# JuliaLinearAlgebra/IterativeSolvers.jl

Hardware: AMD Instinct MI355X
Metric: cg_iters_per_sec (higher is better)
Workload: dtype f64; 1 GPU; cg! on 256^3 3D 7-point Laplacian (test/laplace_matrix.jl), fp64, hashed rhs, x0 = 0 (BASELINE.json configs[1]); n=16777216, nnz=117047296

## Files before the change

iterativesolvers.jl_amd/csrc/mik_core.hip:

```cpp
#include <algorithm>
#include <cmath>
#include <cstdarg>
#include <limits>
#include <new>

#include "mik_kernels.h"
#include "mik_spmv.h"
#include <algorithm>
#include <mutex>

#include "mik_sell.h"
#include "mik_jds.h"
#include <map>
#include <string>
#include <unordered_map>

thread_local std::string g_mik_create_error;
int g_mik_tuning[MIK_KNOB_COUNT] = {0};
static std::vector<mik_ctx *> g_mik_contexts;
static std::mutex g_mik_contexts_mu;

int mik_fail(mik_ctx *ctx, int code, const char *fmt, ...)
{
    char buf[512];
// ... 877 lines not shown
    std::vector<int> rowptr, col;
    std::vector<unsigned char> v;
    if (ctx->tuning[MIK_KNOB_UPLOAD] != 1 && nnz > 0 && n_rows > 0 && n_cols > 0 && n_rows < 0x7f000000) {
        mik_csr *A = new (std::nothrow) mik_csr();
        if (!A) return mik_fail(ctx, MIK_ERR_NOMEM, "mik_csr_create: host allocation failed");
        A->ctx = ctx; A->dtype = dtype; A->n_rows = n_rows; A->n_cols = n_cols; A->nnz = nnz;
        (void)hipSetDevice(ctx->device);
        int rc = mik_upload_device(ctx, A, dtype, n_rows, n_cols, nnz, ptr, idx, val, index_base, is_csc);
        if (rc == MIK_OK && !A->sdia_val && !A->sdia_pats && (ctx->tuning[MIK_KNOB_LAYOUTS] & 1) == 0 && ctx->tuning[MIK_KNOB_UPLOAD] != 2) {
            rc = mik_build_sdiaw_device(ctx, A);
            if (rc == MIK_OK) rc = mik_build_jds_device(ctx, A);
            if (rc == MIK_OK) rc = mik_build_xwin_device(ctx, A);
        } else if (rc == MIK_OK && !A->sdia_val && !A->sdia_pats && (ctx->tuning[MIK_KNOB_LAYOUTS] & 1) == 0) {
            try {
                rowptr.resize((size_t)n_rows + 1);
                col.resize((size_t)nnz);
                v.resize((size_t)nnz * es);
            } catch (const std::bad_alloc &) {
                mik_csr_destroy(A);
                return mik_fail(ctx, MIK_ERR_NOMEM, "mik_csr_create: host staging allocation failed");
            }
            if (hipMemcpy(rowptr.data(), A->rowptr, sizeof(int) * ((size_t)n_rows + 1), hipMemcpyDeviceToHost) != hipSuccess ||
                hipMemcpy(col.data(), A->col, sizeof(int) * (size_t)nnz, hipMemcpyDeviceToHost) != hipSuccess ||
                hipMemcpy(v.data(), A->val, es * (size_t)nnz, hipMemcpyDeviceToHost) != hipSuccess) {
                mik_csr_destroy(A);
                return mik_fail(ctx, MIK_ERR_HIP, "mik_csr_create: reading the device CSR back failed");
            }
            rc = csr_build_sdiaw(ctx, A, rowptr, col, v, es, n_rows, n_cols, nnz);
            if (rc == MIK_OK) rc = csr_build_jds(ctx, A, rowptr, col, v, es, n_rows, nullptr);
            if (rc == MIK_OK) rc = csr_build_xwin(ctx, A, rowptr, col, es, n_rows, n_cols, A->max_row_nnz);
            if (rc == MIK_OK) rc = mik_build_rperm_host(ctx, A, rowptr.data());
        }
        if (rc == MIK_OK) rc = sdiaw_chunk_bits(ctx, A);
        if (rc == MIK_OK) { *out = A; return MIK_OK; }
        mik_csr_destroy(A);
        if (rc != MIK_ERR_NOTIMPL) return rc;
    }
    if (on_device) return MIK_ERR_NOTIMPL;
    try {
        rowptr.assign((size_t)n_rows + 1, 0);
        col.resize((size_t)nnz);
        v.resize((size_t)nnz * es);
    } catch (const std::bad_alloc &) {
        return mik_fail(ctx, MIK_ERR_NOMEM, "mik_csr_create: host staging allocation failed");
    }
    for (int64_t j = 0; j < n_major; ++j)
        if (ptr[j + 1] < ptr[j]) return mik_fail(ctx, MIK_ERR_INVALID, "mik_csr_create: ptr not monotone at %lld", (long long)j);
    for (int64_t k = 0; k < nnz; ++k) {
        const int64_t i = idx[k] - index_base;
        if (i < 0 || i >= n_minor) return mik_fail(ctx, MIK_ERR_INVALID, "mik_csr_create: index %lld out of range at %lld", (long long)idx[k], (long long)k);
    }
    int max_row = 0;
    if (is_csc) {
        for (int64_t k = 0; k < nnz; ++k) rowptr[(size_t)(idx[k] - index_base) + 1]++;
        for (int64_t r = 0; r < n_rows; ++r) {
            max_row = std::max(max_row, rowptr[r + 1]);
            rowptr[r + 1] += rowptr[r];
        }
        std::vector<int> cursor(rowptr.begin(), rowptr.end() - 1);
        for (int64_t j = 0; j < n_cols; ++j)
            for (int64_t k = ptr[j] - index_base; k < ptr[j + 1] - index_base; ++k) {
                const int64_t r = idx[k] - index_base;
                const int dst = cursor[r]++;
                col[dst] = (int)j;
                memcpy(&v[(size_t)dst * es], (const unsigned char *)val + (size_t)k * es, es);
            }
// ... 137 lines not shown
                for (size_t q = 4 * g2; q < std::min(4 * g2 + 4, long_rows.size()); ++q) {
                    lo = std::min<int64_t>(lo, col[(size_t)long_start[q]]);
                    hi = std::max<int64_t>(hi, col[(size_t)long_start[q] + (size_t)long_len[q] - 1]);
                }
                lo &= ~(int64_t)(W - 1);
                if (lo + LW > n_cols) lo = (n_cols - LW) & ~(int64_t)(W - 1);
                if (hi - lo < 2 * LW) { lwin[g2] = (int)lo; ++with_window; }
            }
            A->long_spread = 2 * with_window >= nwg;
            if (!A->long_spread) {
                std::fill(lwin.begin(), lwin.end(), -1);
                std::vector<int> ord(long_rows.size());
                for (size_t q = 0; q < ord.size(); ++q) ord[q] = (int)q;
                std::stable_sort(ord.begin(), ord.end(), [&](int a, int b) { return long_len[(size_t)a] > long_len[(size_t)b]; });
                std::vector<int> tab3;
                for (int q : ord) tab3.push_back(long_rows[(size_t)q]);
                for (int q : ord) tab3.push_back(long_start[(size_t)q]);
                for (int q : ord) tab3.push_back(long_len[(size_t)q]);
                if (hipMemcpy(A->long_rows, tab3.data(), sizeof(int) * tab3.size(), hipMemcpyHostToDevice) != hipSuccess) {
                    cleanup();
                    return mik_fail(ctx, MIK_ERR_HIP, "mik_csr_create: long-row table");
                }
            }
            hipError_t e2;
            if ((e2 = hipMalloc((void **)&A->long_win, sizeof(int) * nwg)) != hipSuccess ||
                (e2 = hipMemcpy(A->long_win, lwin.data(), sizeof(int) * nwg, hipMemcpyHostToDevice)) != hipSuccess) {
                cleanup();
                return mik_fail(ctx, MIK_ERR_HIP, "mik_csr_create: long-row windows: %s", hipGetErrorString(e2));
            }
            A->long_lw = (int)LW;
        }
    }
    if (rc_layout == MIK_OK) rc_layout = sdiaw_chunk_bits(ctx, A);
    if (rc_layout != MIK_OK) { cleanup(); return rc_layout; }
    *out = A;
    return MIK_OK;
}

extern "C" int mik_csr_destroy(mik_csr *A)
{
    if (!A) return MIK_OK;
    if (A->ctx) (void)hipStreamSynchronize(A->ctx->stream);
    if (A->rowptr) (void)hipFree(A->rowptr);
    if (A->col) (void)hipFree(A->col);
    if (A->val) (void)hipFree(A->val);
    if (A->long_rows) (void)hipFree(A->long_rows);
    if (A->is_long) (void)hipFree(A->is_long);
    if (A->seg_sum) (void)hipFree(A->seg_sum);
    if (A->sdia_ptr) (void)hipFree(A->sdia_ptr);
    if (A->sdia_off) (void)hipFree(A->sdia_off);
    if (A->sdia_tri) (void)hipFree(A->sdia_tri);
    if (A->sdia_mask) (void)hipFree(A->sdia_mask);
    if (A->sdia_val) (void)hipFree(A->sdia_val);
    if (A->sdia_pats) (void)hipFree(A->sdia_pats);
    if (A->sdia_pat_id) (void)hipFree(A->sdia_pat_id);
    if (A->sdia_recs) (void)hipFree(A->sdia_recs);
    if (A->sdiaw_pats) (void)hipFree(A->sdiaw_pats);
    if (A->sdiaw_pat_id) (void)hipFree(A->sdiaw_pat_id);
    if (A->sdiaw_mask) (void)hipFree(A->sdiaw_mask);
    if (A->sdiaw_uz) (void)hipFree(A->sdiaw_uz);
    if (A->xwin_lo) (void)hipFree(A->xwin_lo);
    if (A->rperm) (void)hipFree(A->rperm);
    if (A->long_win) (void)hipFree(A->long_win);
    if (A->jds_ptr) (void)hipFree(A->jds_ptr);
    if (A->jds_len) (void)hipFree(A->jds_len);
    if (A->jds_col) (void)hipFree(A->jds_col);
    if (A->jds_val) (void)hipFree(A->jds_val);
    delete A;
    return MIK_OK;
}

static int spmv_kernel_choice(const mik_csr *A);
extern "C" int mik_csr_layout(const mik_csr *A, int *layout)
{
    if (!A || !layout) return MIK_ERR_INVALID;
    *layout = spmv_kernel_choice(A);
// ... 33 lines not shown
    if (!A) return MIK_ERR_INVALID;
    if (n_rows) *n_rows = A->n_rows;
    if (n_cols) *n_cols = A->n_cols;
    if (nnz) *nnz = A->nnz;
    if (dtype) *dtype = A->dtype;
    return MIK_OK;
}

template <typename T>
int mik_spmv_launch_range(mik_ctx *ctx, const mik_csr *A, const T *x, T *y, bool fuse_dot, T *seg_out, const int *done, int rb_begin,
                          int rb_count);

static int spmv_kernel_choice(const mik_csr *A)
{
    const bool csr = A->col != nullptr;
    if (A->force_layout == 0 && csr) return 0;
    if ((A->ctx->tuning[MIK_KNOB_LAYOUTS] & 1) == 0 || !csr) {
        if (A->sdia_pats && ((A->ctx->tuning[MIK_KNOB_LAYOUTS] & 4) == 0 || !csr)) return 5;
        if (A->sdia_val && ((A->ctx->tuning[MIK_KNOB_LAYOUTS] & 4) == 0 || !csr)) return 4;
        if (A->sdiaw_pats && ((A->ctx->tuning[MIK_KNOB_LAYOUTS] & 4) == 0 || !csr)) return 6;
        if (A->jds_val && (A->ctx->tuning[MIK_KNOB_LAYOUTS] & 8) == 0) return 1;
    }
    return 0;
}

extern "C" int mik_csr_compact(mik_csr *A)
{
    if (!A) return MIK_ERR_INVALID;
    if (!A->col) return MIK_OK;
    if (!(A->sdia_pats || A->sdia_val || A->sdiaw_pats || A->jds_val) || A->n_long)
        return mik_fail(A->ctx, MIK_ERR_NOTIMPL, "mik_csr_compact: this operator runs on its CSR arrays");
    if (A->ctx) { (void)hipSetDevice(A->ctx->device); (void)hipStreamSynchronize(A->ctx->stream); }
    (void)hipFree(A->rowptr); (void)hipFree(A->col); (void)hipFree(A->val);
    A->rowptr = nullptr; A->col = nullptr; A->val = nullptr;
    return MIK_OK;
}

static inline bool spmv_csr_rowgather(const mik_csr *A)
{
    return A->ctx->tuning[MIK_KNOB_CSR_KERNEL] == 2 || (A->ctx->tuning[MIK_KNOB_CSR_KERNEL] == 0 && A->n_long == 0 && !A->xwin_lo && !A->rperm);
}

static bool sdiab2_applies(const mik_csr *A)
{
    return A->sdia_buf_ok && A->sdia_cls >= 1 && (A->n_rows & 1) == 0 && A->ctx->tuning[MIK_KNOB_SDIA_KERNEL] == 0;
}

bool mik_spmv_has_epilogue(const mik_csr *A)
{
    if (!A || A->ctx->tuning[MIK_KNOB_SOLVER_FORM] == 2) return false;
    const int kc = spmv_kernel_choice(A);
    if (kc == 5) return A->sdia_buf_ok && A->ctx->tuning[MIK_KNOB_SDIA_KERNEL] != 1 && sdiab2_applies(A);
    return (kc == 0 || kc == 1) && A->n_long == 0;
}

bool mik_spmv_is_light(const mik_csr *A) { return A && (spmv_kernel_choice(A) == 5 || spmv_kernel_choice(A) == 6); }

extern "C" int mik_spmv_kernel(const mik_csr *A, char *name, int len)
{
    if (!A || !name || len <= 0) return MIK_ERR_INVALID;
    const char *k = "k_spmv_rowblock";
    switch (spmv_kernel_choice(A)) {
    case 5: k = A->sdia_buf_ok && A->ctx->tuning[MIK_KNOB_SDIA_KERNEL] != 1 ? (sdiab2_applies(A) ? "k_spmv_sdiab2" : "k_spmv_sdiab") : "k_spmv_sdiac"; break;
    case 6: k = ((A->n_rows & 1) == 0 && A->ctx->tuning[MIK_KNOB_SDIA_KERNEL] != 3) ? "k_spmv_sdiaw2" : "k_spmv_sdiaw"; break;
    case 4: k = "k_spmv_sdia"; break;
    case 1: k = "k_spmv_jds"; break;
    default: k = spmv_csr_rowgather(A) ? "k_spmv_rowgather" : ((A->xwin_lo && (A->ctx->tuning[MIK_KNOB_LAYOUTS] & 96) == 0) ? "k_spmv_rowblock+xwin" : "k_spmv_rowblock"); break;
// ... 157 lines not shown
        lt.seg_sum = A->seg_sum; lt.nlong = nlong;
    }
    const int nlb = (nlong + 3) / 4;
    const int *lwin = (A->long_win && (ctx->tuning[MIK_KNOB_LAYOUTS] & 96) == 0 && mik_aligned16(x)) ? A->long_win : nullptr;
    if (choice == 1) {
        using IV = typename WideVec<T>::idx;
        using VV = typename WideVec<T>::val;
        const bool inside = fuse_dot && nlong == 0;
#define MIK_JDS_GO(FD, NTV, MG)                                                                                                        \
    hipLaunchKernelGGL((k_spmv_jds<T, FD, NTV, MG>), dim3(nb + (MG ? nlb : 0)), dim3(MIK_BLOCK), 0, ctx->stream, n, rb0, A->jds_ptr, A->jds_len, \
                       (const IV *)A->jds_col, (const VV *)A->jds_val, x, y, seg_out, done, nlb, lt, A->col, (const T *)A->val, (const T *)ctx->spmv_ep_w, (const T *)ctx->spmv_ep_c, (const T *)ctx->spmv_ep_z)
#define MIK_JDS_GO2(NTV)                                                                      \
    do {                                                                                      \
        if (inside) MIK_JDS_GO(true, NTV, false);                                             \
        else if (nlong) MIK_JDS_GO(false, NTV, true);                                         \
        else MIK_JDS_GO(false, NTV, false);                                                   \
    } while (0)
        MIK_JDS_GO2(true);
#undef MIK_JDS_GO2
#undef MIK_JDS_GO
        MIK_LAUNCH_CHECK(ctx);
        if (fuse_dot && !inside) {
            hipLaunchKernelGGL((k_rowdot<T>), dim3(nb_all), dim3(MIK_BLOCK), 0, ctx->stream, n, x, (const T *)y, seg_out, done);
            MIK_LAUNCH_CHECK(ctx);
        }
        return MIK_OK;
    }
    if (spmv_csr_rowgather(A)) {
        if (nlong) {
            hipLaunchKernelGGL((k_spmv_longrows<T>), dim3(nlb), dim3(MIK_BLOCK), lwin ? sizeof(T) * (size_t)A->long_lw : 0, ctx->stream, lt, A->col, (const T *)A->val, x, y, done,
                               lwin, A->long_lw);
            MIK_LAUNCH_CHECK(ctx);
        }
#define MIK_RG_GO(FD, NTV)                                                                                                      \
    hipLaunchKernelGGL((k_spmv_rowgather<T, FD, NTV>), dim3(nb), dim3(MIK_BLOCK), 0, ctx->stream, n, rb0, nb, map_mode, A->rowptr, \
                       A->col, (const T *)A->val, x, y, seg_out, done, A->is_long, (const T *)ctx->spmv_ep_w, (const T *)ctx->spmv_ep_c, (const T *)ctx->spmv_ep_z)
        if (fuse_dot) { MIK_RG_GO(true, true); }
        else          { MIK_RG_GO(false, true); }
#undef MIK_RG_GO
        MIK_LAUNCH_CHECK(ctx);
        return MIK_OK;
    }
    const bool merge = nlong > 0 && !fuse_dot;
    const bool nt_rb = !A->xwin_lo;
    if (nlong && !merge) {
        hipLaunchKernelGGL((k_spmv_longrows<T>), dim3(nlb), dim3(MIK_BLOCK), lwin ? sizeof(T) * (size_t)A->long_lw : 0, ctx->stream, lt, A->col, (const T *)A->val, x, y, done,
                           lwin, A->long_lw);
        MIK_LAUNCH_CHECK(ctx);
    }
    const dim3 grid(nb + (merge ? nlb : 0)), block(MIK_BLOCK);
    const bool xwin = A->xwin_lo && wide && (ctx->tuning[MIK_KNOB_LAYOUTS] & 96) == 0 && mik_aligned16(x);
    constexpr int RB_TILE = MIK_SPMV_TILE * (int)(8 / sizeof(T));
    const size_t dyn = sizeof(T) * ((size_t)RB_TILE + 12 + (xwin ? (size_t)A->xwin_span : 0));
    const int lw_launch = (int)std::min<size_t>((size_t)A->long_lw, dyn / 1024 * (1024 / sizeof(T)));
    const bool rp = A->rperm && wide && (ctx->tuning[MIK_KNOB_LAYOUTS] & 96) == 0;
#define MIK_SPMV_GO(FD, NT, WD, MG, XW, RP)                                                                      \
    hipLaunchKernelGGL((k_spmv_rowblock<T, FD, NT, WD, MG, XW, RP>), grid, block, dyn, ctx->stream, n, nb, map_mode, A->rowptr, \
                       A->col, (const T *)A->val, x, y, seg_out, done, A->is_long, nlb, lt, (const int *)A->xwin_lo, A->xwin_span, (const unsigned char *)A->rperm, \
                       MG ? lwin : (const int *)nullptr, (MG && lwin && A->long_spread) ? -lw_launch : lw_launch, (const T *)ctx->spmv_ep_w, (const T *)ctx->spmv_ep_c, (const T *)ctx->spmv_ep_z)
#define MIK_SPMV_GO3(FD, NT, MG)                                                          \
    do {                                                                                  \
        if (xwin) { if (rp) MIK_SPMV_GO(FD, NT, true, MG, true, true); else MIK_SPMV_GO(FD, NT, true, MG, true, false); }   \
        else if (rp) MIK_SPMV_GO(FD, NT, true, MG, false, true);                          \
        else if (wide) MIK_SPMV_GO(FD, NT, true, MG, false, false);                       \
        else MIK_SPMV_GO(FD, NT, false, MG, false, false);                                \
    } while (0)
#define MIK_SPMV_GO2(FD, MG) do { if (nt_rb) MIK_SPMV_GO3(FD, true, MG); else MIK_SPMV_GO3(FD, false, MG); } while (0)
    if (fuse_dot) MIK_SPMV_GO2(true, false);
// ... 357 lines not shown
```

iterativesolvers.jl_amd/csrc/mik_internal.h:

```cpp
#pragma once
#include <hip/hip_runtime.h>

#include <algorithm>
#include <cmath>
#include <cstdint>
#include <cstdio>
#include <cstring>
#include <limits>
#include <string>
#include <vector>

#include "../../include/mik.h"
#include "../../include/mik_dev.h"

constexpr int MIK_BLOCK = 256;
constexpr int MIK_RED_L = 2;
constexpr int MIK_FIN_THREADS = 1024;
constexpr int MIK_SPMV_TILE = 2048;
constexpr int MIK_SPMV_G = 1;
constexpr int MIK_LONG_ROW = 256;
constexpr int MIK_XCD_MAP = 8;

template <typename T> struct VT;
template <> struct VT<double> { static constexpr int W = 2; using vec = double2; };
// ... 18 lines not shown
    const void *spmv_ep_w = nullptr, *spmv_ep_c = nullptr;
    const void *spmv_ep_z = nullptr;
    int tuning[MIK_KNOB_COUNT] = {0};
    static constexpr size_t COEF_BYTES = 8192;
    static constexpr size_t COEF_SAFE_SLOT = 4096;
    std::vector<std::pair<void *, int (*)(void *)>> owned;
};

static inline int mik_cus(const mik_ctx *ctx) { const int v = ctx->tuning[MIK_KNOB_MACHINE] & 0xFFFF; return v > 0 ? v : std::max(1, ctx->cu_count); }
static inline int mik_xcds(const mik_ctx *ctx) { const int v = (ctx->tuning[MIK_KNOB_MACHINE] >> 16) & 0xFF; return v > 0 ? v : std::max(1, ctx->xcd_count); }
static inline bool mik_xcd_maps(const mik_ctx *ctx) { return mik_xcds(ctx) == MIK_XCD_MAP; }
static inline int mik_max_grid(const mik_ctx *ctx) { return mik_cus(ctx) * 32; }
static inline int mik_resident_cap(const mik_ctx *ctx) { return mik_cus(ctx); }
static inline int mik_strip_for(const mik_ctx *ctx, int64_t bw, int64_t nb)
{
    if (!mik_xcd_maps(ctx)) return 0;
    const int64_t P = ((bw + MIK_BLOCK - 1) / MIK_BLOCK + MIK_XCD_MAP - 1) / MIK_XCD_MAP * MIK_XCD_MAP;
    return (P >= MIK_XCD_MAP && P <= nb / 4) ? (int)P : 0;
}

int mik_mgs_resident_max_s();

struct mik_csr {
    mik_ctx *ctx = nullptr;
    int dtype = MIK_F64;
    int64_t n_rows = 0, n_cols = 0, nnz = 0;
    int *rowptr = nullptr;
    int *col = nullptr;
    void *val = nullptr;
    int max_row_nnz = 0;
    int strip = 0;
    int force_layout = -1;
    int max_rowblock_nnz = 0;
    int n_long = 0;
    int *xwin_lo = nullptr;
    int xwin_span = 0;
    int *long_win = nullptr;
    int long_lw = 0;
    bool long_spread = false;
    unsigned char *rperm = nullptr;
    int *long_rows = nullptr;
    int n_seg = 0, n_cut = 0;
    void *seg_sum = nullptr;
    unsigned char *is_long = nullptr;
    void *sdiaw_pats = nullptr;
    int *sdiaw_pat_id = nullptr;
    unsigned *sdiaw_mask = nullptr;
    void *sdiaw_uz = nullptr;
    int sdiaw_npat = 0, sdiaw_koff = 0, sdiaw_pat_bytes = 0;
    int *jds_ptr = nullptr;
    unsigned short *jds_len = nullptr;
    int *jds_col = nullptr;
    void *jds_val = nullptr;
    int64_t jds_groups = 0;
    int64_t jds_short_nnz = 0;
    int *sdia_ptr = nullptr;
    int *sdia_off = nullptr;
    int *sdia_tri = nullptr;
    unsigned char *sdia_mask = nullptr;
    void *sdia_val = nullptr;
    int64_t sdia_entries = 0;
    void *sdia_pats = nullptr;
    int *sdia_pat_id = nullptr;
    int sdia_npat = 0;
    bool sdia_buf_ok = false;
    int sdia_koff = 0;
// ... 29 lines not shown
                      const void *val, int index_base, int is_csc);

int mik_ensure_partials(mik_ctx *ctx, size_t bytes);
int mik_build_sdiaw_device(mik_ctx *ctx, mik_csr *A);
int mik_build_jds_device(mik_ctx *ctx, mik_csr *A);
bool mik_spmv_has_epilogue(const mik_csr *A);
static inline bool mik_xwin_plan(int64_t nb, const int *mn, const int *mx, const int *cnt, size_t es, int64_t n_cols, int64_t total_entries,
                                 std::vector<int> &lo, int *span_out)
{
    const int W = (int)(16 / es), XP = (int)(1024 / es);
    const int64_t cap = 32768 / (int64_t)es - W;
    lo.assign((size_t)nb, 0);
    int64_t need = 0, inside = 0;
    for (int64_t b = 0; b < nb; ++b) {
        if (cnt[b] <= 0) continue;
        lo[(size_t)b] = mn[b] & ~(W - 1);
        const int64_t nd = (int64_t)mx[b] + 1 - lo[(size_t)b];
        if (nd > cap) { lo[(size_t)b] = -1; continue; }
        need = std::max(need, nd);
        inside += cnt[b];
    }
    if (need <= 0 || 4 * inside < 3 * total_entries) return false;
    const int64_t span = (need + W + XP - 1) / XP * XP;
    if (span + W > n_cols) return false;
    for (int64_t b = 0; b < nb; ++b) {
        if (cnt[b] <= 0 || lo[(size_t)b] < 0 || (int64_t)lo[(size_t)b] + span <= n_cols) continue;
        const int64_t slid = (n_cols - span) & ~(int64_t)(W - 1);
        lo[(size_t)b] = slid + span > (int64_t)mx[b] ? (int)slid : -1;
    }
    *span_out = (int)span;
    return true;
}
int mik_build_xwin_device(mik_ctx *ctx, mik_csr *A);
int mik_build_rperm_host(mik_ctx *ctx, mik_csr *A, const int *rowptr_host);

#define MIK_HIP(ctx, call)                                                                    \
    do {                                                                                      \
        hipError_t e_ = (call);                                                               \
        if (e_ != hipSuccess)                                                                 \
            return mik_fail((ctx), e_ == hipErrorOutOfMemory ? MIK_ERR_NOMEM : MIK_ERR_HIP,    \
                            "%s failed: %s (%s:%d)", #call, hipGetErrorString(e_), __FILE__,   \
                            __LINE__);                                                        \
    } while (0)

#define MIK_LAUNCH_CHECK(ctx)                                                                 \
    do {                                                                                      \
        hipError_t e_ = hipGetLastError();                                                    \
        if (e_ != hipSuccess)                                                                 \
            return mik_fail((ctx), MIK_ERR_HIP, "kernel launch failed: %s (%s:%d)",           \
                            hipGetErrorString(e_), __FILE__, __LINE__);                       \
    } while (0)

static inline bool mik_aligned16(const void *p) { return (reinterpret_cast<uintptr_t>(p) & 15u) == 0; }
static inline size_t mik_dtype_size(int dtype) { return dtype == MIK_F64 ? 8 : 4; }

static inline int64_t mik_spmv_nwg(int64_t n)
{
    const int64_t rows = (int64_t)MIK_BLOCK * MIK_SPMV_G;
    return (n + rows - 1) / rows;
}

template <typename T> static inline int64_t mik_nseg(int64_t n)
{
    const int64_t seg = (int64_t)MIK_BLOCK * VT<T>::W * MIK_RED_L;
    return (n + seg - 1) / seg;
}
// ... 232 lines not shown
```

iterativesolvers.jl_amd/csrc/mik_spmv.h:

```cpp
#pragma once
#include "mik_internal.h"

#ifdef __HIPCC__

template <bool NT, typename U> __device__ __forceinline__ U ld_stream(const U *p)
{
    return NT ? __builtin_nontemporal_load(p) : *p;
}
template <bool NT, typename U> __device__ __forceinline__ void st_stream(U *p, U v)
{
    if (NT) __builtin_nontemporal_store(v, p); else *p = v;
}

typedef double mik_f64x2 __attribute__((ext_vector_type(2)));
typedef float mik_f32x4 __attribute__((ext_vector_type(4)));
typedef int mik_i32x2 __attribute__((ext_vector_type(2)));
typedef int mik_i32x4 __attribute__((ext_vector_type(4)));
template <typename T> struct WideVec;
template <> struct WideVec<double> { using val = mik_f64x2; using idx = mik_i32x2; };
template <> struct WideVec<float>  { using val = mik_f32x4; using idx = mik_i32x4; };

__device__ __forceinline__ int spmv_block_map(int b, int nb, int mode)
{
    if (mode == 1) return xcd_remap(b, nb);
    if (mode >= 8) {
        const int P = mode, S = P >> 3;
        if (b < (nb / P) * P) {
            const int xcd = b & 7, q = b >> 3;
            return (q / S) * P + xcd * S + (q % S);
        }
    }
    return b;
}

constexpr int MIK_LONG_G = 4;

constexpr int MIK_LONG_SEG = 1024;

struct LongTab {
    const int *rows, *starts, *lens;
    const int *seg_row;
    const int *cut_row, *cut_first, *cut_nseg;
    unsigned *tickets;
    void *seg_sum;
    int nlong;
};

template <typename T> __device__ __forceinline__ void longrow_store(const LongTab &lt, int w, T acc, T *__restrict__ y)
{
    const int lane = threadIdx.x & 63;
    const int tgt = lt.rows[w];
    if (tgt >= 0) { if (lane == 0) y[tgt] = acc; return; }
    const int sg = -tgt - 1;
    T *ss = (T *)lt.seg_sum;
    const int h = lt.seg_row[sg];
    const int ns = lt.cut_nseg[h];
    int last = 0;
    if (lane == 0) {
        __hip_atomic_store(&ss[sg], acc, __ATOMIC_RELAXED, __HIP_MEMORY_SCOPE_AGENT);
// ... 230 lines not shown
            for (int i = 0; i < 8; ++i) q[i] = prod[a + i];
#pragma unroll
            for (int i = 0; i < 8; ++i) acc = acc + q[i];
        }
        if (len > 0) {
            T q[8];
#pragma unroll
            for (int i = 0; i < 8; ++i) q[i] = prod[a + i];
#pragma unroll
            for (int i = 0; i < 8; ++i) {
                const T s2 = acc + q[i];
                acc = i < len ? s2 : acc;
            }
        }
        __syncthreads();
    }
    if (FUSE_DOT && ep_w && r < n) { const T te = *ep_c * ep_w[r]; acc = acc + te; }
    if (is_long && r < n && is_long[r]) acc = y[r];
    else if (r < n) st_stream<NT>(y + r, acc);
    if (FUSE_DOT) {
        T p = T(0);
        if (r < n) p = (ep_z ? ep_z[r] : x[r]) * acc;
        if (RPERM) {
            prod[tr] = p;
            __syncthreads();
            p = prod[t];
        }
        T tot = block_tree_256(p, lds4);
        if (t == 0) seg_out[rb] = tot;
    }
}

template <typename T, bool FUSE_DOT, bool NT>
__global__ __launch_bounds__(MIK_BLOCK, 6) void k_spmv_rowgather(int n, int rb0, int nb, int map_mode, const int *__restrict__ rowptr,
                                                              const int *__restrict__ col, const T *__restrict__ val,
                                                              const T *__restrict__ x, T *__restrict__ y, T *__restrict__ seg_out,
                                                              const int *__restrict__ done, const unsigned char *__restrict__ is_long,
                                                              const T *__restrict__ ep_w = nullptr, const T *__restrict__ ep_c = nullptr,
                                                             const T *__restrict__ ep_z = nullptr)
{
    if (done && *done) return;
    constexpr int TILE = MIK_SPMV_TILE;
    constexpr int VW = VT<T>::W;
    constexpr int VP = 1024 / (int)sizeof(T);
    constexpr int CP = 256;
    __shared__ __attribute__((aligned(16))) T sval[TILE];
    __shared__ __attribute__((aligned(16))) int scol[TILE];
    __shared__ T lds4[4];

    const int t = threadIdx.x, lane = t & 63, wv = t >> 6;
    const int rb = rb0 + spmv_block_map((int)blockIdx.x, nb, map_mode);
    const int r0 = rb * MIK_BLOCK;
    const int r = r0 + t;
    int ks = 0, ke = 0;
    if (r < n) { ks = rowptr[r]; ke = rowptr[r + 1]; }
    const int kb = rowptr[r0] & ~3;
    const int kend = rowptr[min(r0 + MIK_BLOCK, n)];

    T acc = T(0);
    for (int kc = kb; kc < kend; kc += TILE) {
        const int cnt = min(TILE, kend - kc);
#pragma unroll
        for (int p = 0; p < TILE / VP / 4; ++p) {
            const int piece = wv + 4 * p;
            if (piece * VP < cnt)
                __builtin_amdgcn_global_load_lds((const __attribute__((address_space(1))) void *)(val + kc + piece * VP + lane * VW),
                                                 (__attribute__((address_space(3))) void *)(sval + piece * VP), 16, 0, NT ? 2 : 0);
        }
#pragma unroll
        for (int p = 0; p < TILE / CP / 4; ++p) {
            const int piece = wv + 4 * p;
            if (piece * CP < cnt)
                __builtin_amdgcn_global_load_lds((const __attribute__((address_space(1))) void *)(col + kc + piece * CP + lane * 4),
                                                 (__attribute__((address_space(3))) void *)(scol + piece * CP), 16, 0, NT ? 2 : 0);
        }
        asm volatile("s_waitcnt vmcnt(0)" ::: "memory");
        __syncthreads();
        int a = max(ks, kc) - kc;
        int len = min(ke, kc + cnt) - kc - a;
        while (len > 0) {
            T q[8];
            int cc[8];
#pragma unroll
            for (int i = 0; i < 8; ++i) {
                const int s = min(a + i, TILE - 1);
                cc[i] = scol[s];
                q[i] = sval[s];
            }
#pragma unroll
            for (int i = 0; i < 8; ++i) {
                const T xv = x[i < len ? cc[i] : 0];
                q[i] = q[i] * xv;
            }
#pragma unroll
            for (int i = 0; i < 8; ++i)
                if (i < len) acc = acc + q[i];
            a += 8;
            len -= 8;
        }
        if (kc + TILE < kend) __syncthreads();
    }
    if (FUSE_DOT && ep_w && r < n) { const T te = *ep_c * ep_w[r]; acc = acc + te; }
    if (is_long && r < n && is_long[r]) acc = y[r];
    else if (r < n) st_stream<NT>(y + r, acc);
    if (FUSE_DOT) {
        T p = T(0);
        if (r < n) p = (ep_z ? ep_z[r] : x[r]) * acc;
        T tot = block_tree_256(p, lds4);
        if (t == 0) seg_out[rb] = tot;
    }
}

#endif
```

iterativesolvers.jl_amd/csrc/mik_upload.hip:

```cpp
#include "mik_internal.h"
#include "mik_sell.h"
#include "mik_jds.h"

#include <algorithm>
#include <cstring>
#include <map>
#include <vector>

namespace {

constexpr int NO_ROW = 0x7f7f7f7f;

struct UploadStats {
    int bad_ptr, bad_idx, dup, max_row, max_rb, sdia_bad, not_constant, pad_;
    long long bw, slots;
};

constexpr int SCAN_PER = 8;
constexpr int SCAN_TILE = MIK_BLOCK * SCAN_PER;

__global__ __launch_bounds__(MIK_BLOCK) void k_scan_tiles(int *__restrict__ data, long long n, int *__restrict__ sums)
{
    __shared__ int part[MIK_BLOCK];
    const int t = threadIdx.x;
// ... 109 lines not shown
    const long long r = (long long)blockIdx.x * blockDim.x + threadIdx.x;
    if (r <= n_rows) rowptr[r] = (int)(ptr[r] - base);
}

__global__ __launch_bounds__(MIK_BLOCK) void k_up_stats(const int *__restrict__ rowptr, const int *__restrict__ col, long long n_rows, UploadStats *st)
{
    const long long r = (long long)blockIdx.x * MIK_BLOCK + threadIdx.x;
    int len = 0;
    long long bw = 0;
    if (r < n_rows) {
        const int a = rowptr[r], b = rowptr[r + 1];
        len = b - a;
        for (int k = a; k < b; ++k)
            if (col[k] < n_rows) bw = max(bw, (long long)llabs((long long)col[k] - r));
    }
    __shared__ int slen[MIK_BLOCK];
    __shared__ long long sbw[MIK_BLOCK];
    slen[threadIdx.x] = len;
    sbw[threadIdx.x] = bw;
    __syncthreads();
    for (int d = MIK_BLOCK / 2; d > 0; d >>= 1) {
        if (threadIdx.x < d) {
            slen[threadIdx.x] = max(slen[threadIdx.x], slen[threadIdx.x + d]);
            sbw[threadIdx.x] = max(sbw[threadIdx.x], sbw[threadIdx.x + d]);
        }
        __syncthreads();
    }
    if (threadIdx.x == 0) {
        atomicMax(&st->max_row, slen[0]);
        atomicMax((unsigned long long *)&st->bw, (unsigned long long)sbw[0]);
        const long long r0 = (long long)blockIdx.x * MIK_BLOCK;
        atomicMax(&st->max_rb, rowptr[min(r0 + MIK_BLOCK, n_rows)] - rowptr[r0]);
    }
}

__global__ void k_up_slice_pattern(const int *__restrict__ rowptr, const int *__restrict__ col, long long n_rows, long long nb, int *__restrict__ doff,
                                   int *__restrict__ dtri, int *__restrict__ nslot, UploadStats *st)
{
    const long long b = (long long)blockIdx.x * blockDim.x + threadIdx.x;
    if (b >= nb) return;
    int offs8[8];
    int ns = 0;
    bool ok = true;
    const long long rend = min((b + 1) * MIK_BLOCK, n_rows);
    for (long long r = b * MIK_BLOCK; r < rend && ok; ++r) {
        int p = 0;
        for (int k2 = rowptr[r]; k2 < rowptr[r + 1]; ++k2) {
            const int d = col[k2] - (int)r;
            int q = 0;
            while (q < ns && offs8[q] != d) ++q;
            if (q < ns) {
                if (q < p) { ok = false; break; }
                p = q + 1;
            } else {
                if (ns == 8) { ok = false; break; }
                for (int z = ns; z > p; --z) offs8[z] = offs8[z - 1];
                offs8[p] = d;
                ++ns;
                ++p;
            }
        }
    }
    if (!ok) { st->sdia_bad = 1; ns = 0; }
    int tri = -1;
    for (int q = 0; q < 8; ++q) doff[b * 8 + q] = q < ns ? offs8[q] : 0;
    for (int q = 0; q + 2 < ns; ++q)
// ... 218 lines not shown
                    UP_TRY(hipMalloc(&A->sdia_val, es * (size_t)std::max(slots_total, 1)));
                    UP_TRY(hipMemsetAsync(A->sdia_val, 0, es * (size_t)std::max(slots_total, 1), st));
                    hipLaunchKernelGGL((k_up_row_values<T>), dim3(blocks_for(n_rows)), dim3(MIK_BLOCK), 0, st, A->rowptr, A->col, (const T *)A->val, (long long)n_rows,
                                       doff, dptr, (T *)A->sdia_val);
                    UP_TRY(hipStreamSynchronize(st));
                    A->sdia_ptr = dptr; A->sdia_off = doff; A->sdia_tri = dtri; A->sdia_mask = mask;
                    S.keep(dptr); S.keep(doff); S.keep(dtri); S.keep(mask);
                    A->sdia_entries = slots_total;
                }
            }
        }
    }
    UP_TRY(hipGetLastError());
    return MIK_OK;
hip_fail:
    rc = (e == hipErrorOutOfMemory) ? MIK_ERR_NOTIMPL
                                    : mik_fail(ctx, MIK_ERR_HIP, "mik_csr_create (device upload): %s", hipGetErrorString(e));
give_up:
    (void)hipStreamSynchronize(st);
    (void)hipGetLastError();
    return rc;
#undef UP_TRY
}

}

int mik_upload_device(mik_ctx *ctx, mik_csr *A, int dtype, int64_t n_rows, int64_t n_cols, int64_t nnz, const int64_t *ptr, const int64_t *idx,
                      const void *val, int index_base, int is_csc)
{
    if (dtype == MIK_F64) return upload_device_t<double>(ctx, A, n_rows, n_cols, nnz, ptr, idx, val, index_base, is_csc);
    return upload_device_t<float>(ctx, A, n_rows, n_cols, nnz, ptr, idx, val, index_base, is_csc);
}

namespace {

struct SdiawDesc { int ns, pad_; int d[32]; unsigned long long bits[32]; };
struct WideStats { int fail; int pad_; };

template <typename T> __device__ __forceinline__ unsigned long long value_bits(T v);
template <> __device__ __forceinline__ unsigned long long value_bits<double>(double v) { return __builtin_bit_cast(unsigned long long, v); }
template <> __device__ __forceinline__ unsigned long long value_bits<float>(float v) { return (unsigned long long)__builtin_bit_cast(unsigned, v); }
template <typename T> __device__ __forceinline__ bool value_finite(T v) { return v - v == T(0); }

template <typename T>
__global__ void k_up_wide_desc(const int *__restrict__ rowptr, const int *__restrict__ col, const T *__restrict__ val, long long n_rows, long long nb,
                               SdiawDesc *__restrict__ desc, WideStats *st)
{
    const long long b = (long long)blockIdx.x * blockDim.x + threadIdx.x;
    if (b >= nb || st->fail) return;
    int d[32];
    unsigned long long bits[32];
    int ns = 0;
    const long long r0 = b * MIK_BLOCK, r1 = r0 + MIK_BLOCK < n_rows ? r0 + MIK_BLOCK : n_rows;
    for (long long r = r0; r < r1; ++r)
        for (int k = rowptr[r]; k < rowptr[r + 1]; ++k) {
            const int dd = col[k] - (int)r;
            const T v = val[k];
            int q = 0;
            while (q < ns && d[q] != dd) ++q;
            if (q == ns) {
                if (ns == 32 || !value_finite(v)) { st->fail = 1; return; }
                d[ns] = dd; bits[ns] = value_bits<T>(v); ++ns;
            } else if (bits[q] != value_bits<T>(v)) { st->fail = 1; return; }
        }
    for (int i = 1; i < ns; ++i) {
        const int dk = d[i];
// ... 291 lines not shown
```

Measured before the change: 2171 iters/s.

## Size row-gather SpMV LDS tile to the largest row-block span using a block pointer table

Builds a per-row-block nonzero pointer table at matrix creation and records the largest block span. The CSR row-gather kernel then uses dynamic LDS sized to that span instead of a fixed tile, and raises its launch bound from 6 to 7 waves for more occupancy. It also hoists the done-flag, row-pointer and dot-operand loads ahead of the tile loop, and adds a shift-based fast path for power-of-two block remapping. Costs are an extra device array, a synchronous build step at creation, and more complex guard logic in the kernel.

```diff
diff --git a/iterativesolvers.jl_amd/csrc/mik_core.hip b/iterativesolvers.jl_amd/csrc/mik_core.hip
--- a/iterativesolvers.jl_amd/csrc/mik_core.hip
+++ b/iterativesolvers.jl_amd/csrc/mik_core.hip
@@ -933,6 +933,7 @@
             if (rc == MIK_OK) rc = mik_build_rperm_host(ctx, A, rowptr.data());
         }
         if (rc == MIK_OK) rc = sdiaw_chunk_bits(ctx, A);
+        if (rc == MIK_OK) rc = mik_build_blk_ptr(ctx, A);
         if (rc == MIK_OK) { *out = A; return MIK_OK; }
         mik_csr_destroy(A);
         if (rc != MIK_ERR_NOTIMPL) return rc;
@@ -1136,6 +1137,7 @@
         }
     }
     if (rc_layout == MIK_OK) rc_layout = sdiaw_chunk_bits(ctx, A);
+    if (rc_layout == MIK_OK) rc_layout = mik_build_blk_ptr(ctx, A);
     if (rc_layout != MIK_OK) { cleanup(); return rc_layout; }
     *out = A;
     return MIK_OK;
@@ -1146,6 +1148,7 @@
     if (!A) return MIK_OK;
     if (A->ctx) (void)hipStreamSynchronize(A->ctx->stream);
     if (A->rowptr) (void)hipFree(A->rowptr);
+    if (A->blk_ptr) (void)hipFree(A->blk_ptr);
     if (A->col) (void)hipFree(A->col);
     if (A->val) (void)hipFree(A->val);
     if (A->long_rows) (void)hipFree(A->long_rows);
@@ -1245,7 +1248,8 @@
         return mik_fail(A->ctx, MIK_ERR_NOTIMPL, "mik_csr_compact: this operator runs on its CSR arrays");
     if (A->ctx) { (void)hipSetDevice(A->ctx->device); (void)hipStreamSynchronize(A->ctx->stream); }
     (void)hipFree(A->rowptr); (void)hipFree(A->col); (void)hipFree(A->val);
-    A->rowptr = nullptr; A->col = nullptr; A->val = nullptr;
+    if (A->blk_ptr) (void)hipFree(A->blk_ptr);
+    A->rowptr = nullptr; A->col = nullptr; A->val = nullptr; A->blk_ptr = nullptr;
     return MIK_OK;
 }
 
@@ -1469,8 +1473,10 @@
                                lwin, A->long_lw);
             MIK_LAUNCH_CHECK(ctx);
         }
+        const int rg_tile = A->rg_tile;
+        const size_t rg_lds = mik_spmv_rowgather_lds<T>(rg_tile);
 #define MIK_RG_GO(FD, NTV)                                                                                                      \
-    hipLaunchKernelGGL((k_spmv_rowgather<T, FD, NTV>), dim3(nb), dim3(MIK_BLOCK), 0, ctx->stream, n, rb0, nb, map_mode, A->rowptr, \
+    hipLaunchKernelGGL((k_spmv_rowgather<T, FD, NTV>), dim3(nb), dim3(MIK_BLOCK), rg_lds, ctx->stream, n, rb0, nb, map_mode, rg_tile, A->blk_ptr, A->rowptr, \
                        A->col, (const T *)A->val, x, y, seg_out, done, A->is_long, (const T *)ctx->spmv_ep_w, (const T *)ctx->spmv_ep_c, (const T *)ctx->spmv_ep_z)
         if (fuse_dot) { MIK_RG_GO(true, true); }
         else          { MIK_RG_GO(false, true); }
diff --git a/iterativesolvers.jl_amd/csrc/mik_internal.h b/iterativesolvers.jl_amd/csrc/mik_internal.h
--- a/iterativesolvers.jl_amd/csrc/mik_internal.h
+++ b/iterativesolvers.jl_amd/csrc/mik_internal.h
@@ -74,6 +74,8 @@
     int strip = 0;
     int force_layout = -1;
     int max_rowblock_nnz = 0;
+    int *blk_ptr = nullptr;
+    int rg_tile = MIK_SPMV_TILE;
     int n_long = 0;
     int *xwin_lo = nullptr;
     int xwin_span = 0;
@@ -169,6 +171,7 @@
     return true;
 }
 int mik_build_xwin_device(mik_ctx *ctx, mik_csr *A);
+int mik_build_blk_ptr(mik_ctx *ctx, mik_csr *A);
 int mik_build_rperm_host(mik_ctx *ctx, mik_csr *A, const int *rowptr_host);
 
 #define MIK_HIP(ctx, call)                                                                    \
diff --git a/iterativesolvers.jl_amd/csrc/mik_spmv.h b/iterativesolvers.jl_amd/csrc/mik_spmv.h
--- a/iterativesolvers.jl_amd/csrc/mik_spmv.h
+++ b/iterativesolvers.jl_amd/csrc/mik_spmv.h
@@ -25,6 +25,11 @@
     if (mode == 1) return xcd_remap(b, nb);
     if (mode >= 8) {
         const int P = mode, S = P >> 3;
+        if ((S & (S - 1)) == 0) {
+            const int sh = __builtin_ctz(S);
+            if (b >= (nb >> (sh + 3)) << (sh + 3)) return b;
+            return (((b >> 3) >> sh) << (sh + 3)) + ((b & 7) << sh) + ((b >> 3) & (S - 1));
+        }
         if (b < (nb / P) * P) {
             const int xcd = b & 7, q = b >> 3;
             return (q / S) * P + xcd * S + (q % S);
@@ -321,58 +326,67 @@
 }
 
 template <typename T, bool FUSE_DOT, bool NT>
-__global__ __launch_bounds__(MIK_BLOCK, 6) void k_spmv_rowgather(int n, int rb0, int nb, int map_mode, const int *__restrict__ rowptr,
+__global__ __launch_bounds__(MIK_BLOCK, 7) void k_spmv_rowgather(int n, int rb0, int nb, int map_mode, int tile, const int *__restrict__ blk_ptr,
+                                                              const int *__restrict__ rowptr,
                                                               const int *__restrict__ col, const T *__restrict__ val,
                                                               const T *__restrict__ x, T *__restrict__ y, T *__restrict__ seg_out,
                                                               const int *__restrict__ done, const unsigned char *__restrict__ is_long,
                                                               const T *__restrict__ ep_w = nullptr, const T *__restrict__ ep_c = nullptr,
-                                                             const T *__restrict__ ep_z = nullptr)
-{
-    if (done && *done) return;
-    constexpr int TILE = MIK_SPMV_TILE;
+                                                              const T *__restrict__ ep_z = nullptr)
+{
     constexpr int VW = VT<T>::W;
     constexpr int VP = 1024 / (int)sizeof(T);
     constexpr int CP = 256;
-    __shared__ __attribute__((aligned(16))) T sval[TILE];
-    __shared__ __attribute__((aligned(16))) int scol[TILE];
-    __shared__ T lds4[4];
+    extern __shared__ __attribute__((aligned(16))) unsigned char mik_dyn_lds[];
+    T *sval = reinterpret_cast<T *>(mik_dyn_lds);
+    int *scol = reinterpret_cast<int *>(sval + tile);
+    T *lds4 = reinterpret_cast<T *>(scol + tile);
 
     const int t = threadIdx.x, lane = t & 63, wv = t >> 6;
     const int rb = rb0 + spmv_block_map((int)blockIdx.x, nb, map_mode);
     const int r0 = rb * MIK_BLOCK;
     const int r = r0 + t;
-    int ks = 0, ke = 0;
-    if (r < n) { ks = rowptr[r]; ke = rowptr[r + 1]; }
-    const int kb = rowptr[r0] & ~3;
-    const int kend = rowptr[min(r0 + MIK_BLOCK, n)];
+    asm volatile("" : : "s"(col), "s"(val));
+    const int rc = min(r, n - 1);
+    int stop = *(done ? done : blk_ptr);
+    const int k0 = blk_ptr[rb];
+    const int kend = blk_ptr[rb + 1];
+    int ks = rowptr[rc], ke = rowptr[rc + 1];
+    T xr = T(0);
+    if (FUSE_DOT) xr = (ep_z ? ep_z : x)[rc];
+    __builtin_amdgcn_sched_barrier(0);
+    if (!done) stop = 0;
+    const int kb = k0 & ~3;
 
     T acc = T(0);
-    for (int kc = kb; kc < kend; kc += TILE) {
-        const int cnt = min(TILE, kend - kc);
-#pragma unroll
-        for (int p = 0; p < TILE / VP / 4; ++p) {
+    int kc = kb;
+    do {
+        const int cnt = max(0, min(tile, kend - kc));
+#pragma unroll
+        for (int p = 0; p < MIK_SPMV_TILE / VP / 4; ++p) {
             const int piece = wv + 4 * p;
-            if (piece * VP < cnt)
+            if (piece * VP + lane * VW < cnt)
                 __builtin_amdgcn_global_load_lds((const __attribute__((address_space(1))) void *)(val + kc + piece * VP + lane * VW),
                                                  (__attribute__((address_space(3))) void *)(sval + piece * VP), 16, 0, NT ? 2 : 0);
         }
 #pragma unroll
-        for (int p = 0; p < TILE / CP / 4; ++p) {
+        for (int p = 0; p < MIK_SPMV_TILE / CP / 4; ++p) {
             const int piece = wv + 4 * p;
-            if (piece * CP < cnt)
+            if (piece * CP + lane * 4 < cnt)
                 __builtin_amdgcn_global_load_lds((const __attribute__((address_space(1))) void *)(col + kc + piece * CP + lane * 4),
                                                  (__attribute__((address_space(3))) void *)(scol + piece * CP), 16, 0, NT ? 2 : 0);
         }
-        asm volatile("s_waitcnt vmcnt(0)" ::: "memory");
+        asm volatile("s_waitcnt vmcnt(0)" : "+v"(ks), "+v"(ke) : : "memory");
         __syncthreads();
+        if (stop) return;
         int a = max(ks, kc) - kc;
-        int len = min(ke, kc + cnt) - kc - a;
+        int len = r < n ? min(ke, kc + cnt) - kc - a : 0;
         while (len > 0) {
             T q[8];
             int cc[8];
 #pragma unroll
             for (int i = 0; i < 8; ++i) {
-                const int s = min(a + i, TILE - 1);
+                const int s = min(a + i, tile - 1);
                 cc[i] = scol[s];
                 q[i] = sval[s];
             }
@@ -387,17 +401,24 @@
             a += 8;
             len -= 8;
         }
-        if (kc + TILE < kend) __syncthreads();
-    }
+        kc += tile;
+        if (kc < kend) __syncthreads();
+    } while (kc < kend);
     if (FUSE_DOT && ep_w && r < n) { const T te = *ep_c * ep_w[r]; acc = acc + te; }
-    if (is_long && r < n && is_long[r]) acc = y[r];
-    else if (r < n) st_stream<NT>(y + r, acc);
+    bool own = r < n;
+    if (is_long) {
+        if (own && is_long[r]) { acc = y[r]; own = false; }
+    }
+    if (!FUSE_DOT) { if (own) st_stream<NT>(y + r, acc); }
     if (FUSE_DOT) {
-        T p = T(0);
-        if (r < n) p = (ep_z ? ep_z[r] : x[r]) * acc;
+        T p = r < n ? xr * acc : T(0);
+        asm volatile("" : "+v"(p) : : "memory");
+        if (own) st_stream<NT>(y + r, acc);
         T tot = block_tree_256(p, lds4);
         if (t == 0) seg_out[rb] = tot;
     }
 }
 
+template <typename T> static inline size_t mik_spmv_rowgather_lds(int tile) { return (size_t)tile * (sizeof(T) + sizeof(int)) + 4 * sizeof(T); }
+
 #endif
diff --git a/iterativesolvers.jl_amd/csrc/mik_upload.hip b/iterativesolvers.jl_amd/csrc/mik_upload.hip
--- a/iterativesolvers.jl_amd/csrc/mik_upload.hip
+++ b/iterativesolvers.jl_amd/csrc/mik_upload.hip
@@ -165,6 +165,15 @@
         const long long r0 = (long long)blockIdx.x * MIK_BLOCK;
         atomicMax(&st->max_rb, rowptr[min(r0 + MIK_BLOCK, n_rows)] - rowptr[r0]);
     }
+}
+
+__global__ void k_up_blk_ptr(const int *__restrict__ rowptr, long long n_rows, long long nb, int *__restrict__ blk_ptr, int *__restrict__ span)
+{
+    const long long b = (long long)blockIdx.x * blockDim.x + threadIdx.x;
+    if (b > nb) return;
+    const int k0 = rowptr[min(b * MIK_BLOCK, n_rows)];
+    blk_ptr[b] = k0;
+    if (b < nb) atomicMax(span, rowptr[min((b + 1) * MIK_BLOCK, n_rows)] - (k0 & ~3));
 }
 
 __global__ void k_up_slice_pattern(const int *__restrict__ rowptr, const int *__restrict__ col, long long n_rows, long long nb, int *__restrict__ doff,
@@ -449,6 +458,27 @@
     return upload_device_t<float>(ctx, A, n_rows, n_cols, nnz, ptr, idx, val, index_base, is_csc);
 }
 
+int mik_build_blk_ptr(mik_ctx *ctx, mik_csr *A)
+{
+    if (!A->rowptr) return MIK_OK;
+    const long long nb = (A->n_rows + MIK_BLOCK - 1) / MIK_BLOCK;
+    int *span = nullptr, hspan = 0;
+    (void)hipSetDevice(ctx->device);
+    MIK_HIP(ctx, hipMalloc((void **)&A->blk_ptr, sizeof(int) * ((size_t)nb + 2)));
+    MIK_HIP(ctx, hipMalloc((void **)&span, sizeof(int)));
+    hipError_t e = hipMemsetAsync(span, 0, sizeof(int), ctx->stream);
+    if (e == hipSuccess) {
+        hipLaunchKernelGGL(k_up_blk_ptr, dim3(blocks_for(nb + 1)), dim3(MIK_BLOCK), 0, ctx->stream, (const int *)A->rowptr, (long long)A->n_rows, nb, A->blk_ptr, span);
+        e = hipGetLastError();
+    }
+    if (e == hipSuccess) e = hipMemcpyAsync(&hspan, span, sizeof(int), hipMemcpyDeviceToHost, ctx->stream);
+    if (e == hipSuccess) e = hipStreamSynchronize(ctx->stream);
+    (void)hipFree(span);
+    if (e != hipSuccess) return mik_fail(ctx, MIK_ERR_HIP, "mik_csr_create: row-block bounds: %s", hipGetErrorString(e));
+    A->rg_tile = std::min(MIK_SPMV_TILE, std::max(4, (hspan + 3) & ~3));
+    return MIK_OK;
+}
+
 namespace {
 
 struct SdiawDesc { int ns, pad_; int d[32]; unsigned long long bits[32]; };
```

New measurement: 2194 iters/s, median of 6. 1.1% higher.
